# traupach/xarray_parcel

Hardware: AMD Instinct MI355X
Metric: column-profiles/sec for surface_based_cape_cin (higher is better)
Workload: dtype f64; 1 GPU; c2: synthetic 64-level x 1024 x 1024 f64 soundings per GPU, 64 levels x 1 x 1024 x 1024, surface_based_cape_cin (CAPE/CIN only), moist mode family, inputs resident in HBM; columns_total=1048576, columns_this_rank=1048576, levels=64, multi_gpu=single GPU

## Files before the change

### xarray_parcel_amd/csrc/xp_device.hpp

```cpp
#pragma once
#include <hip/hip_runtime.h>
#include <stdint.h>

namespace xp {

constexpr double RD = 287.04749097718457;
constexpr double EPS = 0.6219569100577033;
constexpr double KAPPA = 2.0 / 7.0;
constexpr double CP_D = RD / KAPPA;
constexpr double LV = 2.50084e6;
constexpr double G = 9.80665;
constexpr double VT_EPS = 0.608;
constexpr double RK4_H_MAX = 0.1;
constexpr double LCL_SNAP = 1e-11;

#define XP_DEV __device__ __forceinline__

XP_DEV double qnan() { return __longlong_as_double(0x7ff8000000000000LL); }
XP_DEV bool isnan_(double x) { return x != x; }
XP_DEV bool isclose_(double x, double y) { return fabs(x - y) <= 1e-8 + 1e-5 * fabs(y); }

constexpr int ST_TOP_NAN = 1, ST_LCL_NOT_CONVERGED = 2, ST_NAN_PRESSURE = 4, ST_BAD_PRESSURE = 8, ST_NO_LAYER = 16,
              ST_BAD_HEIGHT = 32, ST_LAYER_OPEN = 64;

// ... 273 lines not shown
    double es_td = es_ref(td);
    double w = EPS * es_td / (p_start - es_td);
    double p0 = p_start, p = qnan();
    bool conv = false;
    for (int it = 0; it < 50; ++it) {
        double td1 = log(p0 * w / (EPS + w) / 6.112); td1 = 273.15 + 243.5 * td1 / (17.67 - td1);
        double p1 = p_start * pow(td1 / t, 1.0 / KAPPA);
        double td2 = log(p1 * w / (EPS + w) / 6.112); td2 = 273.15 + 243.5 * td2 / (17.67 - td2);
        double p2 = p_start * pow(td2 / t, 1.0 / KAPPA);
        double d = p2 - 2.0 * p1 + p0;
        p = (d != 0.0) ? p0 - (p1 - p0) * (p1 - p0) / d : p2;
        double rel = (p0 != 0.0) ? (p - p0) / p0 : p;
        if (fabs(rel) < 1e-5) { conv = true; break; }
        p0 = p;
    }
    if (!conv) { p = qnan(); r.not_converged = 1; }
    if (fabs(p - p_start) <= 1e-8 + 1e-5 * fabs(p_start)) p = p_start;
    r.p = p;
    double v = log(p * w / (EPS + w) / 6.112);
    r.t = 273.15 + 243.5 * v / (17.67 - v);
    r.tv = virt_ref(r.t, r.t, p);
    return r;
}
__device__ __attribute__((noinline)) Lcl lcl_reference(double p_start, double t, double td) { return lcl_reference_body(p_start, t, td); }
template <bool FLAT = false> XP_DEV Lcl lcl(double p_start, double t, double td) {
    Lcl r;
    r.not_converged = 0;
    if (isnan_(p_start) || isnan_(t) || isnan_(td)) { r.p = r.t = r.tv = qnan(); return r; }
    bool sane = (td <= t) && (td > 150.0) && (t < 350.0) && (p_start > 50.0) && (p_start < 1200.0);
    double es_td = sat_vapor_pressure(td);
    double w = EPS * fdiv(es_td, p_start - es_td);
    double p0 = p_start, p = qnan();
    bool conv = false;
    for (int it = 0; it < 50; ++it) {
        double p1 = lcl_iter(p0, p_start, w, t);
        double p2 = lcl_iter(p1, p_start, w, t);
        double d = p2 - 2.0 * p1 + p0;
        p = (d != 0.0) ? p0 - fdiv((p1 - p0) * (p1 - p0), d) : p2;
        double rel = (p0 != 0.0) ? fdiv(p - p0, p0) : p;
        if (fabs(rel) < 1e-5) { conv = true; break; }
        p0 = p;
        if (!sane) break;
    }
    if (!conv) { p = qnan(); r.not_converged = 1; }
    if (fabs(p - p_start) <= 1e-8 + 1e-5 * fabs(p_start)) p = p_start;
    r.p = p;
    r.t = dewpoint_fast(p * fdiv(w, EPS + w));
    r.tv = virt(r.t, mix_of_e(sat_vapor_pressure(r.t), p));
    bool ref_path = !sane || (p == p_start);
    if (__builtin_amdgcn_ballot_w64(ref_path) != 0ull && ref_path) r = FLAT ? lcl_reference_body(p_start, t, td) : lcl_reference(p_start, t, td);
    return r;
}

XP_DEV double dt_dlnp_e(double p, double t, double e) {
    double pe = p - e, rt2 = RD * t * t;
    double num = __builtin_fma(RD * t, pe, (LV * EPS) * e);
    double den = __builtin_fma(CP_D * rt2, pe, (LV * LV * EPS * EPS) * e);
    return rt2 * fdiv(num, den);
}
XP_DEV double dt_dlnp(const double *es, double p, double t, bool fast) { return dt_dlnp_e(p, t, es_tab(es, t, fast)); }

struct Tables {
    const uint16_t *index;
    const float *adiabats;
    int64_t n_p, n_t;
    double p_max, p_step, t_min, t_step;
};

struct Moist {
    double x, p, t, e;
    const float *row;
    const double *es;
    bool table, dead;

    XP_DEV void start(const double *es_lds, double p_ref, double x_ref, double t_ref, bool table_mode, const Tables &tb) {
        es = es_lds; x = x_ref; p = p_ref; t = t_ref; table = table_mode; row = nullptr;
        e = es_tab(es, t_ref);
        dead = isnan_(p_ref) || isnan_(t_ref);
        if (table_mode && !dead) {
            double fi = (tb.p_max - p_ref) / tb.p_step, fj = (t_ref - tb.t_min) / tb.t_step;
            double i0 = floor(fi), j0 = floor(fj);
            int64_t ip = (int64_t)(((i0 + 1.0) - fi < fi - i0) ? i0 + 1.0 : i0);
            int64_t jt = (int64_t)(((j0 + 1.0) - fj <= fj - j0) ? j0 + 1.0 : j0);
            ip = ip < 0 ? 0 : (ip > tb.n_p - 1 ? tb.n_p - 1 : ip);
            jt = jt < 0 ? 0 : (jt > tb.n_t - 1 ? tb.n_t - 1 : jt);
            uint16_t a = tb.index[ip * tb.n_t + jt];
            if (a) row = tb.adiabats + (int64_t)(a - 1) * tb.n_p;
        }
    }
    XP_DEV double at(double pk, double xk, const Tables &tb, bool hoist = false) {
        if (dead || isnan_(pk)) return qnan();
        if (table) {
            double p_min = tb.p_max - (double)(tb.n_p - 1) * tb.p_step;
            if (row == nullptr || pk < p_min || pk > tb.p_max) return qnan();
            double f = (pk - p_min) / tb.p_step;
            int64_t lo = (int64_t)floor(f);
            if (lo >= tb.n_p - 1) return (double)row[tb.n_p - 1];
            double xlo = p_min + (double)lo * tb.p_step, xhi = p_min + (double)(lo + 1) * tb.p_step;
            double ylo = (double)row[lo], yhi = (double)row[lo + 1];
            return (yhi - ylo) / (xhi - xlo) * (pk - xlo) + ylo;
        }
        if (xk != x) {
            double dx = xk - x;
            int ns = (int)ceil(fabs(dx) * (1.0 / RK4_H_MAX) - 1e-12);
            ns = ns < 1 ? 1 : ns;
            double h = dx * frcp((double)ns);
            double q = 0.5 * h;
            double rh = 2.48015873015873e-05;
            rh = __builtin_fma(rh, q, 1.984126984126984e-04);
            rh = __builtin_fma(rh, q, 1.388888888888889e-03);
            rh = __builtin_fma(rh, q, 8.333333333333333e-03);
            rh = __builtin_fma(rh, q, 4.1666666666666664e-02);
            rh = __builtin_fma(rh, q, 1.6666666666666666e-01);
            rh = __builtin_fma(rh, q, 0.5);
            rh = __builtin_fma(rh, q, 1.0);
            rh = __builtin_fma(rh, q, 1.0);
            double ps = p;
            for (int s = 0; s < ns; ++s) {
                double pm = ps * rh;
                double pe = (s == ns - 1) ? pk : pm * rh;
                bool fast = hoist && (__builtin_amdgcn_ballot_w64(!in_table(t, 10.0)) == 0ull);
                double k1 = dt_dlnp_e(ps, t, e);
                double k2 = dt_dlnp(es, pm, t + 0.5 * h * k1, fast);
                double k3 = dt_dlnp(es, pm, t + 0.5 * h * k2, fast);
                double k4 = dt_dlnp(es, pe, t + h * k3, fast);
                t = t + (h * (1.0 / 6.0)) * (k1 + 2.0 * k2 + 2.0 * k3 + k4);
                e = es_tab(es, t, fast);
                ps = pe;
            }
            x = xk; p = pk;
        }
        return t;
    }
};

constexpr double FAM_XHI = 7.003065458786462;
constexpr double FAM_WX = 0.5, FAM_X1000 = 6.907755278982137;
constexpr int FAM_NPX = 8, FAM_ND = 8, FAM_MD = 8, FAM_NPS = 9;
constexpr double FAM_XLO = FAM_XHI - FAM_WX * FAM_NPX;
constexpr int FAM_COEFS = FAM_NPX * (FAM_ND + 1) * (FAM_MD + 1) * FAM_NPS;
constexpr int FAM_SIZE = FAM_COEFS + 2 * FAM_NPS;
constexpr double FAM_LABEL_H = 0.25, FAM_MARGIN = 0.05;
constexpr double FAM_PSI_LO = 215.0, FAM_PSI_HI = 312.0;
#define XP_FAM_EDGES {215.0, 245.0, 262.0, 275.0, 285.0, 293.0, 299.0, 304.0, 308.5, 312.0}

constexpr int FAM_SM = (FAM_ND + 1) * FAM_NPX * FAM_NPS, FAM_SN = FAM_NPX * FAM_NPS, FAM_SJ = FAM_NPS;
struct Family {
    const double *tab;
    double c[FAM_ND + 1];
    double m4;
    double s;
    int q;
    bool bad;

    XP_DEV static int psi_piece(double psi) {
        return (int)(psi >= 245.0) + (int)(psi >= 262.0) + (int)(psi >= 275.0) + (int)(psi >= 285.0) + (int)(psi >= 293.0) +
               (int)(psi >= 299.0) + (int)(psi >= 304.0) + (int)(psi >= 308.5);
    }
    XP_DEV static double x_mid(int j) { return FAM_XHI - FAM_WX * ((double)j + 0.5); }
    XP_DEV void load_piece(int j) {
        const double *a = tab + (j * FAM_SJ + q);
#pragma unroll
        for (int n = 0; n <= FAM_ND; ++n) {
            const double *r = a + n * FAM_SN;
            double k[FAM_MD + 1];
#pragma unroll
            for (int m = 0; m <= FAM_MD; ++m) k[m] = r[m * FAM_SM];
            lds_wait_all();
            double v = k[FAM_MD];
#pragma unroll
            for (int m = FAM_MD - 1; m >= 0; --m) v = __builtin_fma(v, s, k[m]);
            asm volatile("" : "+v"(v) : : "memory");
            c[n] = v;
        }
        m4 = -(2.0 / FAM_WX) * x_mid(j);
    }
    XP_DEV static double temperature_of(const double *es, double p, double tv) {
        constexpr double c = VT_EPS * EPS;
        double e0 = es_tab(es, tv);
        double t = fdiv(tv, 1.0 + c * fdiv(e0, p - e0));
#pragma nounroll
        for (int it = 0; it < 5; ++it) {
            double e = es_tab(es, t);
            double rt = frcp(t - 29.65), rp = frcp(p - e);
            double de = e * (17.67 * 243.5) * (rt * rt);
            double g = c * e * rp;
            double f = __builtin_fma(t, g, t) - tv;
            double df = 1.0 + g + t * c * p * de * (rp * rp);
            t = t - fdiv(f, df);
        }
        return t;
    }
    XP_DEV static double temperature_from(const double *es, double p, double tv, double &off, bool all_in_range = false) {
        constexpr double c = VT_EPS * EPS;
        double t = tv - off, f = 0.0;
#pragma nounroll
        for (int it = 0; it < 3; ++it) {
            double e = es_tab(es, t, all_in_range);
#ifdef XP_NEWTON_EXACT_SLOPE
            double rt = frcp(t - 29.65), rp = frcp(p - e);
#else
            double rt = __builtin_amdgcn_rcp(t - 29.65), rp = frcp(p - e);
#endif
            double de = e * (17.67 * 243.5) * (rt * rt);
            double g = c * e * rp;
            f = __builtin_fma(t, g, t) - tv;
            double df = 1.0 + g + t * c * p * de * (rp * rp);
#ifdef XP_NEWTON_EXACT_SLOPE
            t = t - fdiv(f, df);
#else
            t = t - f * __builtin_amdgcn_rcp(df);
#endif
        }
        bool more = !(fabs(f) <= 1e-6);
        if (__builtin_amdgcn_ballot_w64(more && !isnan_(tv)) != 0ull) {
#pragma nounroll
            for (int it = 0; it < 2; ++it) {
                double e = es_tab(es, t);
                double rt = frcp(t - 29.65), rp = frcp(p - e);
                double de = e * (17.67 * 243.5) * (rt * rt);
                double g = c * e * rp;
                double f2 = __builtin_fma(t, g, t) - tv;
                double df = 1.0 + g + t * c * p * de * (rp * rp);
                t = more ? t - fdiv(f2, df) : t;
            }
        }
        if (!isnan_(t)) off = tv - t;
        return t;
    }
    XP_DEV static double temperature_from2(const double *es, double p, double tv, double &off, double &offp, bool all_in_range) {
        constexpr double c = VT_EPS * EPS;
        double t = tv - (2.0 * off - offp), f = 0.0;
#pragma nounroll
        for (int it = 0; it < 2; ++it) {
            double e = es_tab(es, t, all_in_range);
            double rt = __builtin_amdgcn_rcp(t - 29.65), rp = frcp(p - e);
            double de = e * (17.67 * 243.5) * (rt * rt);
            double g = c * e * rp;
            f = __builtin_fma(t, g, t) - tv;
            double df = 1.0 + g + t * c * p * de * (rp * rp);
            t = t - f * __builtin_amdgcn_rcp(df);
        }
        bool more = !(fabs(f) <= 3e-5);
        if (__builtin_amdgcn_ballot_w64(more && !isnan_(tv)) != 0ull) {
#pragma nounroll
            for (int it = 0; it < 2; ++it) {
                double e = es_tab(es, t);
                double rt = frcp(t - 29.65), rp = frcp(p - e);
                double de = e * (17.67 * 243.5) * (rt * rt);
                double g = c * e * rp;
                double f2 = __builtin_fma(t, g, t) - tv;
                double df = 1.0 + g + t * c * p * de * (rp * rp);
                t = more ? t - fdiv(f2, df) : t;
            }
        }
        if (!isnan_(t)) { offp = off; off = tv - t; }
        return t;
    }
    XP_DEV double horner(double z) const {
        double v = c[FAM_ND];
#pragma unroll
        for (int n = FAM_ND - 1; n >= 0; --n) v = __builtin_fma(v, z, c[n]);
        return v;
    }
    XP_DEV void start(const double *table, const double *es, double p_lcl, double x_lcl, double t_lcl, double tv_lcl) {
        tab = table; q = 0; s = 0.0; m4 = 0.0;
        bad = !(x_lcl >= FAM_XLO && x_lcl <= FAM_XHI) || isnan_(t_lcl);
        double dx = FAM_X1000 - x_lcl;
        int ns = (int)ceil(fabs(dx) * (1.0 / FAM_LABEL_H) - 1e-12);
        ns = ns < 1 ? 1 : ns;
        ns = bad ? 1 : ns;
        double h = bad ? 0.0 : dx * frcp((double)ns);
        double qh = 0.5 * h;
        double rh = 2.755731922398589e-07;
        rh = __builtin_fma(rh, qh, 2.7557319223985893e-06);
        rh = __builtin_fma(rh, qh, 2.48015873015873e-05);
        rh = __builtin_fma(rh, qh, 1.984126984126984e-04);
        rh = __builtin_fma(rh, qh, 1.388888888888889e-03);
        rh = __builtin_fma(rh, qh, 8.333333333333333e-03);
        rh = __builtin_fma(rh, qh, 4.1666666666666664e-02);
        rh = __builtin_fma(rh, qh, 1.6666666666666666e-01);
        rh = __builtin_fma(rh, qh, 0.5);
        rh = __builtin_fma(rh, qh, 1.0);
        rh = __builtin_fma(rh, qh, 1.0);
        double t = t_lcl, ps = p_lcl;
#pragma nounroll
        for (int k = 0; k < ns; ++k) {
            double pm = ps * rh, pe = pm * rh;
            double k1 = dt_dlnp(es, ps, t, false);
            double k2 = dt_dlnp(es, pm, t + 0.5 * h * k1, false);
            double k3 = dt_dlnp(es, pm, t + 0.5 * h * k2, false);
            double k4 = dt_dlnp(es, pe, t + h * k3, false);
            t = t + (h * (1.0 / 6.0)) * (k1 + 2.0 * k2 + 2.0 * k3 + k4);
            ps = pe;
        }
        const double psi0 = t;
        if (!(psi0 >= FAM_PSI_LO + FAM_MARGIN && psi0 <= FAM_PSI_HI - FAM_MARGIN)) bad = true;
        q = bad ? 0 : psi_piece(psi0);
        const double mid = tab[FAM_COEFS + q], inv_h = tab[FAM_COEFS + FAM_NPS + q];
        double u = __builtin_fma(-(1.0 / FAM_WX), x_lcl, FAM_XHI * (1.0 / FAM_WX));
        int j0 = bad ? 0 : (int)u;
        j0 = j0 > FAM_NPX - 1 ? FAM_NPX - 1 : j0;
        const double z = bad ? 0.0 : (x_lcl - x_mid(j0)) * (2.0 / FAM_WX);
        const double *a = tab + (j0 * FAM_SJ + q);
        double b[FAM_MD + 1];
#pragma unroll
        for (int m = 0; m <= FAM_MD; ++m) {
            double k[FAM_ND + 1];
#pragma unroll
            for (int n = 0; n <= FAM_ND; ++n) k[n] = a[m * FAM_SM + n * FAM_SN];
            lds_wait_all();
            double v = k[FAM_ND];
#pragma unroll
            for (int n = FAM_ND - 1; n >= 0; --n) v = __builtin_fma(v, z, k[n]);
            asm volatile("" : "+v"(v) : : "memory");
            b[m] = v;
        }
        double psi = psi0;
#pragma unroll
        for (int it = 0; it < 3; ++it) {
            double sc = (psi - mid) * inv_h;
            double val = 0.0, der = 0.0;
#pragma unroll
            for (int m = FAM_MD; m >= 0; --m) {
                der = __builtin_fma(der, sc, val);
                val = __builtin_fma(val, sc, b[m]);
            }
            psi = psi - fdiv(val - tv_lcl, der * inv_h);
        }
        if (!(fabs(psi - psi0) <= FAM_MARGIN)) bad = true;
        s = bad ? 0.0 : (psi - mid) * inv_h;
        load_piece(j0);
        if (bad) poison();
    }
    XP_DEV double locate(double X, bool &top, bool &any_top) {
        double z = __builtin_fma(2.0 / FAM_WX, X, m4);
        top = false; any_top = false;
        bool move = (z <= -1.0) || (z > 1.0);
        if (__builtin_amdgcn_ballot_w64(move) != 0ull) {
            double u = __builtin_fma(-(1.0 / FAM_WX), X, FAM_XHI * (1.0 / FAM_WX));
            bool go = move;
            if (go && u < 0.0) { bad = true; go = false; }
            int jn = (int)u;
            top = go && jn > FAM_NPX - 1;
            int jcur = (int)__builtin_rint(__builtin_fma(m4, 0.5, FAM_XHI * (1.0 / FAM_WX) - 0.5));
            int j = go ? (jn > FAM_NPX - 1 ? FAM_NPX - 1 : jn) : jcur;
            load_piece(bad ? 0 : j);
            if (bad) poison();
            z = __builtin_fma(2.0 / FAM_WX, X, m4);
            any_top = __builtin_amdgcn_ballot_w64(top) != 0ull;
        }
        return z;
    }
    XP_DEV double top_value(double v, double X, bool top) const {
        const double w = horner(-1.0);
        return top ? w * fexp(KAPPA * (X - FAM_XLO)) : v;
    }
    XP_DEV double at(double X) {
        double z = __builtin_fma(2.0 / FAM_WX, X, m4);
        bool move = (z <= -1.0) || (z > 1.0);
        if (__builtin_amdgcn_ballot_w64(move) != 0ull) {
            double u = __builtin_fma(-(1.0 / FAM_WX), X, FAM_XHI * (1.0 / FAM_WX));
            bool go = move;
            if (go && u < 0.0) { bad = true; go = false; }
            int jn = (int)u;
            bool top = go && jn > FAM_NPX - 1;
            int jcur = (int)__builtin_rint(__builtin_fma(m4, 0.5, FAM_XHI * (1.0 / FAM_WX) - 0.5));
            int j = go ? (jn > FAM_NPX - 1 ? FAM_NPX - 1 : jn) : jcur;
            load_piece(bad ? 0 : j);
            if (bad) poison();
            z = __builtin_fma(2.0 / FAM_WX, X, m4);
            if (__builtin_amdgcn_ballot_w64(top) != 0ull) {
                double v = horner(top ? -1.0 : z);
                return top ? v * fexp(KAPPA * (X - FAM_XLO)) : v;
            }
        }
        return horner(z);
    }
    XP_DEV void poison() {
#pragma unroll
        for (int n = 0; n <= FAM_ND; ++n) c[n] = qnan();
        m4 = qnan();
    }
};

#ifndef XP_CAPE_THREADS
#define XP_CAPE_THREADS 256
#endif
#ifndef XP_SLOT_FIELDS
#define XP_SLOT_FIELDS (XP_CAPE_THREADS >= 1024 ? 12 : 13)
#endif
constexpr int SLOT_STRIDE = XP_CAPE_THREADS, SLOT_FIELDS = XP_SLOT_FIELDS;
enum { SL_CAPE_LCL = 0, SL_CIN_LCL, SL_MIN_P, SL_IDX , SL_LCL_T,
       SL_A0, SL_A1, SL_A2, SL_A3, SL_EL_X, SL_EL_T, SL_CAPE_EL, SL_LI ,
       SL_BR_P = SL_A0, SL_BR_X = SL_A1, SL_BR_T = SL_A2, SL_BR_TD = SL_A3,
       SL_LFC_X = SL_A0, SL_LFC_T = SL_A1, SL_CAPE_LFC = SL_A2, SL_CIN_LFC = SL_A3 };

struct Scan {
    double p_lcl, x_lcl;
    bool pos_neg;
    double *slot;
    double Xp, yp, parp;
    int j;
    bool use_all;
    double cape, cin;
    int any_inc;
    bool pos_parcel, env_any;
    bool top_le, any_valid;
    bool bad_p;

    XP_DEV void init(double p_lcl_, double x_lcl_, bool pos_neg_, double *slot_) {
        p_lcl = p_lcl_; x_lcl = x_lcl_; pos_neg = pos_neg_; slot = slot_;
        Xp = yp = parp = qnan(); j = 0; use_all = true;
        cape = cin = 0.0;
        for (int f = 0; f < SLOT_FIELDS; ++f)
            slot[f * SLOT_STRIDE] = (f == SL_LFC_T || f == SL_EL_T || f == SL_LFC_X || f == SL_EL_X || f == SL_MIN_P || f == SL_LI) ? qnan() : 0.0;
        idx()[0] = -1; idx()[1] = -1;
        any_inc = 0;
        pos_parcel = env_any = top_le = any_valid = bad_p = false;
    }
    XP_DEV int *idx() const { return (int *)(slot + SL_IDX * SLOT_STRIDE); }
    XP_DEV void add(double a) {
        if (pos_neg) { cape += fmax(a, 0.0); cin += fmin(a, 0.0); }
        else { double b = isnan_(a) ? 0.0 : a; cape += b; cin += b; }
    }
    XP_DEV double crossing_pressure(double xs) const {
        double ps = fexp(xs);
        bool near_lcl = fabs(xs - x_lcl) <= 2e-9;
        if (__builtin_amdgcn_ballot_w64(near_lcl) != 0ull && near_lcl) {
            double q = xs;
            asm volatile("" : "+v"(q));
            ps = exp_slow(q);
        }
        return ps;
    }
    template <bool LEAN, bool ABOVE> XP_DEV void special(double X, double par, double env, double y, double a_reg) {
        if (!ABOVE && j == 0) { use_all = (env != par); return; }
        int i = j - 1;
        double d = y - yp, xs, frac;
        if constexpr (ABOVE) {
            const double r = frcp1(d);
            xs = (y * Xp - yp * X) * r;
            if (isnan_(xs)) return;
            frac = -yp * r;
            add((yp * 0.5) * fabs(Xp - xs));
            if (y > 0.0) {
                any_inc = 1;
                if (!(xs <= slot[SL_LFC_X * SLOT_STRIDE])) {
                    slot[SL_LFC_X * SLOT_STRIDE] = xs; if (!LEAN) idx()[0] = j - 1;
                    if (!LEAN) slot[SL_LFC_T * SLOT_STRIDE] = frac * (par - parp) + parp;
                    slot[SL_CAPE_LFC * SLOT_STRIDE] = cape; slot[SL_CIN_LFC * SLOT_STRIDE] = cin;
                }
            }
            if (y < 0.0 && !(xs >= slot[SL_EL_X * SLOT_STRIDE])) {
                slot[SL_EL_X * SLOT_STRIDE] = xs; if (!LEAN) idx()[1] = j - 1;
                if (!LEAN) slot[SL_EL_T * SLOT_STRIDE] = frac * (par - parp) + parp;
                slot[SL_CAPE_EL * SLOT_STRIDE] = cape;
            }
            add((y * 0.5) * fabs(X - xs));
            return;
        }
        bool dup = (X == Xp);
        if (__builtin_amdgcn_ballot_w64(dup) != 0ull && dup) {
            xs = (y * Xp - yp * X) / d;
            frac = (xs - Xp) / (X - Xp);
        } else {
            double r = frcp1(d);
            xs = (y * Xp - yp * X) * r;
            frac = -yp * r;
        }
        double zy = frac * d + yp;
        if (isnan_(zy)) { add(a_reg); return; }
        double zlog = xs;
        bool above = ABOVE || xs < x_lcl;
        bool near_lcl = !ABOVE && fabs(xs - x_lcl) <= 2e-9;
        if (!ABOVE && __builtin_amdgcn_ballot_w64(near_lcl) != 0ull && near_lcl) {
            double q = y;
            asm volatile("" : "+v"(q));
            xs = crossing_x_ref(q, yp, X, Xp);
            double ps = exp_slow(xs);
            zlog = log_slow(ps);
            above = ps < p_lcl;
        }
        add((yp * 0.5) * fabs(Xp - zlog));
        double ys = frac * (par - parp) + parp;
        if (!isnan_(xs)) {
            bool in_sel = ABOVE || use_all || i >= 1;
            if (y > 0.0 && in_sel) {
                any_inc = 1;
                if (above && !(xs <= slot[SL_LFC_X * SLOT_STRIDE])) {
                    slot[SL_LFC_X * SLOT_STRIDE] = xs; if (!LEAN) idx()[0] = i;
                    if (!LEAN) slot[SL_LFC_T * SLOT_STRIDE] = ys;
                    slot[SL_CAPE_LFC * SLOT_STRIDE] = cape; slot[SL_CIN_LFC * SLOT_STRIDE] = cin;
                }
            }
            if (y < 0.0 && (ABOVE || i >= 1) && above && !(xs >= slot[SL_EL_X * SLOT_STRIDE])) {
                slot[SL_EL_X * SLOT_STRIDE] = xs; if (!LEAN) idx()[1] = i;
                if (!LEAN) slot[SL_EL_T * SLOT_STRIDE] = ys;
                slot[SL_CAPE_EL * SLOT_STRIDE] = cape;
            }
        }
        add((y * 0.5) * fabs(X - zlog));
    }
    template <bool LEAN = false, bool ABOVE = false> XP_DEV void node(double P, double X, double par, double env, bool is_lcl) {
        if (is_lcl) {
            slot[SL_LFC_X * SLOT_STRIDE] = qnan(); slot[SL_LFC_T * SLOT_STRIDE] = qnan();
            slot[SL_CAPE_LFC * SLOT_STRIDE] = 0.0; slot[SL_CIN_LFC * SLOT_STRIDE] = 0.0;
        }
        asm volatile("" : "+v"(par), "+v"(env));
        double y = par - env;
        bool same = (y * yp > 0.0) | ((y == 0.0) & (yp == 0.0));
        double a = fabs(X - Xp) * ((yp + y) * 0.5);
        add(same ? a : 0.0);
#ifdef XP_NODE_BALLOT
        if (__builtin_amdgcn_ballot_w64(!same) != 0ull && !same) special<LEAN, ABOVE>(X, par, env, y, a);
#else
        if (!same) special<LEAN, ABOVE>(X, par, env, y, a);
#endif
        pos_parcel = pos_parcel || ((ABOVE || P < p_lcl) && par > env);
        if (!LEAN) {
            bad_p = bad_p || (X > Xp);
            env_any = env_any || !isnan_(env);
        }
        bool pv = (ABOVE && LEAN) || !isnan_(P);
        bool valid = pv && !isnan_(par) && !isnan_(env);
        if (!LEAN && pv) slot[SL_MIN_P * SLOT_STRIDE] = P;
        top_le = (valid & (par <= env)) | (!valid & top_le);
        if (!LEAN) any_valid = any_valid || valid;
        if (is_lcl) { slot[SL_CAPE_LCL * SLOT_STRIDE] = cape; slot[SL_CIN_LCL * SLOT_STRIDE] = cin; }
        Xp = X; yp = y; parp = par; ++j;
// ... 44 lines not shown
```

### xarray_parcel_amd/csrc/xp_kernels.hpp

```cpp
#pragma once
#include "xp_level_reader.hpp"
#include "xp_profile_out.hpp"

namespace xp {

struct CapeArgs {
    View p, t, td;
    int64_t nlev, ncol;
    const void *ex_p, *ex_t, *ex_td;
    double depth;
    int vtc, log_interp, pos_neg, post_zero, table_mode;
    int hum;
    int off32;
    Tables tb;
    const double *es_tab;
    const double *fam_tab;
    int32_t *flags;
    int persist;
    int only_flagged;
    ScalarsOut s;
    ProfileOut prof;
};

enum { PM_SURFACE = 0, PM_MU = 1, PM_ML = 2, PM_EXPLICIT = 3 };
// ... 102 lines not shown
        if (!isnan_(p) && p < top) {
            double lt = flog(top), cb = flog(pb), ca = flog(p);
            double th_a = t / fpow(p / 1000.0, KAPPA), w_a = sat_mix(p, td);
            double cb2 = cb, ca2 = ca, tha = th_a, wa = w_a;
            if (pb == top) { ca2 = cb; tha = thb; wa = wb; }
            double th_t = interp_rule(thb, tha, lt, cb2, ca2), w_t = interp_rule(wb, wa, lt, cb2, ca2);
            layer_mean_step(s_th, pp, thp, top, th_t);
            layer_mean_step(s_w, pp, wp, top, w_t);
            r.first = k; closed = true;
            break;
        }
        double th = t / fpow(p / 1000.0, KAPPA), w = sat_mix(p, td);
        if (k > 0) { layer_mean_step(s_th, pp, thp, p, th); layer_mean_step(s_w, pp, wp, p, w); }
        pp = p; thp = th; wp = w;
        if (!isnan_(p)) { pb = p; thb = th; wb = w; }
    }
    if (!closed) {
        double th_t = (pb == top) ? thb : qnan(), w_t = (pb == top) ? wb : qnan();
        layer_mean_step(s_th, pp, thp, top, th_t);
        layer_mean_step(s_w, pp, wp, top, w_t);
    }
    double dlay = fabs(top - bottom);
    double th_m = (1.0 / dlay) * s_th, w_m = (1.0 / dlay) * s_w;
    r.p = p_start;
    r.t = th_m * fpow(p_start / 1000.0, KAPPA);
    r.td = dewpoint_of_e(vapor_pressure(p_start, w_m));
    return r;
}

template <typename T, bool HUM> XP_DEV Parcel choose_parcel(const CapeArgs &a, int pmode, int64_t c, const double *es, const double depth) {
    Parcel pc;
    if (pmode == PM_SURFACE) {
        pc.p = ld<T>(a.p, 0, c); pc.t = ld<T>(a.t, 0, c); pc.td = as_dewpoint<HUM>(es, pc.p, pc.t, ld<T>(a.td, 0, c));
        pc.first = 0; pc.idx = 0; pc.prepend = false;
    } else if (pmode == PM_EXPLICIT) {
        pc.p = ld1<T>(a.ex_p, c); pc.t = ld1<T>(a.ex_t, c); pc.td = ld1<T>(a.ex_td, c);
        pc.first = 0; pc.idx = -1; pc.prepend = false;
    } else if (pmode == PM_MU) {
        pc = select_mu<T, HUM>(a, c, es, depth);
    } else {
        pc = select_ml<T, HUM>(a, c, es, depth);
    }
    return pc;
}

template <typename T, int PMODE, bool PROFILE, int MODE, bool HUM, bool DEF, bool LEAN, bool PERSIST>
__global__ __launch_bounds__(XP_CAPE_THREADS, (XP_CAPE_THREADS >= 1024 ? 4 : MODE == 2 ? 3 : PROFILE ? 4 : (PMODE == PM_SURFACE ? (HUM ? 3 : 1) : 4))) void k_cape_cin(CapeArgs a) {
    constexpr bool TABLE = (MODE == 1), FAMILY = (MODE == 2);
    constexpr bool LAZY = FAMILY && PROFILE && LEAN;
    struct Lds { double es[LDS_TAB]; double fam[FAMILY ? FAM_SIZE : 1]; double slot[SLOT_FIELDS * SLOT_STRIDE]; int next; };
    struct LdsRef { double *es, *fam, *slot; int *next; } lds;
    if constexpr (FAMILY && PROFILE) {
        __shared__ double l_es[LDS_TAB];
        __shared__ double l_fam[FAM_SIZE];
        __shared__ double l_slot[SLOT_FIELDS * SLOT_STRIDE];
        __shared__ int l_next;
        lds.es = l_es; lds.fam = l_fam; lds.slot = l_slot; lds.next = &l_next;
    } else {
        __shared__ Lds l;
        lds.es = l.es; lds.fam = l.fam; lds.slot = l.slot; lds.next = &l.next;
    }
    double *const s_es = lds.es;
    double *const s_fam = lds.fam;
    if (FAMILY) for (int i = threadIdx.x; i < FAM_SIZE; i += blockDim.x) s_fam[i] = a.fam_tab[i];
    int &s_next = *lds.next;
    if (PERSIST && threadIdx.x == 0) s_next = (int)(blockDim.x >> 6);
    int64_t c0 = (int64_t)blockIdx.x * blockDim.x + threadIdx.x;
    if (a.only_flagged) {
        int need = (c0 < a.ncol) ? a.flags[c0] : 0;
        if (!__syncthreads_or(need)) return;
        stage_es_table(a.es_tab, s_es);
        if (!need) return;
    } else {
        stage_es_table(a.es_tab, s_es);
        if (!PERSIST && c0 >= a.ncol) return;
    }
    const double *es = s_es;
    double *const s_slot = lds.slot;

    auto column = [&](const int64_t c) __attribute__((always_inline)) {
    const Parcel pc = choose_parcel<T, HUM>(a, PMODE, c, es, a.depth);

    const bool vtc = DEF || (a.vtc != 0), pos_neg = DEF || (a.pos_neg != 0), log_interp = DEF || (a.log_interp != 0);
    const bool need_w = vtc || PROFILE;
    const Lcl l = lcl(pc.p, pc.t, pc.td);
    int status = l.not_converged ? ST_LCL_NOT_CONVERGED : 0;
    const ScalarsOut &s = a.s;

    if (isnan_(l.p)) {
        if (PROFILE) ProfileSink<T, LAZY>::blank(a.prof, c);
        store_blank_column(s, c, pc, l, status);
        if (FAMILY) a.flags[c] = 0;
        return;
    }

    store_parcel_and_lcl(s, c, pc, l);
    const double vf_parcel = need_w ? virt_factor_tab(es, pc.t, pc.td, pc.p, false) : 1.0;
    const double x_lcl = log(l.p);
    const double x0 = (pc.p == l.p) ? x_lcl : log_tab<true>(es, pc.p);

    Scan sc; sc.init(l.p, x_lcl, pos_neg, s_slot + threadIdx.x);
    sc.slot[SL_LCL_T * SLOT_STRIDE] = vtc ? l.tv : l.t;
    Moist m;
    Family fam;
    if (FAMILY) fam.start(s_fam, es, l.p, x_lcl, l.t, l.tv);
    else m.start(es, l.p, x_lcl, l.t, TABLE, a.tb);
    double fam_off = l.tv - l.t;
    double fam_offp = fam_off;

    ProfileSink<T, LAZY> sink;
    constexpr bool TRACK = LEAN && PMODE == PM_ML;
    int last_k = -1, cur_k = -1;
    auto emit = [&](auto above, double P, double X, double tp, double tvp, double te, double tve, double tde, bool is_lcl) __attribute__((always_inline)) {
        if (PROFILE) sink.node(a.prof, c, es, sc, P, X, tp, tvp, te, tve, tde);
        if (TRACK) {
            if (!isnan_(P)) { last_k = (is_lcl || cur_k < 0) ? -1 : cur_k; if (is_lcl || cur_k < 0) sc.slot[SL_MIN_P * SLOT_STRIDE] = P; }
        }
        sc.template node<LEAN, decltype(above)::value>(P, X, vtc ? tvp : tp, vtc ? tve : te, is_lcl);
    };

    bool lcl_done = false;
    double *const br = sc.slot;
    clear_bracket(br);
    auto moist_node = [&](double P, double X, double T_, double m_, bool Q) __attribute__((always_inline)) {
        constexpr bool TRIO = FAMILY && LEAN && !PROFILE && !HUM && (PMODE == PM_SURFACE || PMODE == PM_EXPLICIT);
        bool f_top = false, f_any_top = false;
        const double fz = TRIO ? fam.locate(X, f_top, f_any_top) : 0.0;
        double tf = TRIO ? 0.0 : FAMILY ? fam.at(X) : m.at(P, X, a.tb, true);
        constexpr bool PARCEL_ES = TABLE;
        constexpr bool FAM_T = FAMILY && PROFILE;
        unsigned dist = table_dist(T_);
        if (!Q) dist = umax_(dist, table_dist(m_));
        if (PARCEL_ES && need_w) dist = umax_(dist, table_dist(tf));
        const bool in_range = all_in_table(dist) && (!FAM_T || LAZY || in_table(tf, 8.0));
        double ep = 0.0, tve, tpf = 0.0;
        if (__builtin_amdgcn_ballot_w64(!in_range) == 0ull) {
            if (need_w && !FAMILY) ep = PARCEL_ES ? es_tab(es, tf, true) : m.e;
            if constexpr (TRIO) {
                double e_td, e_t;
                es_tab2_horner(es, m_, T_, fam.c, fz, e_td, e_t, tf);
                tve = T_ * __builtin_fma(e_td * frcp1(P - e_t), VT_EPS * EPS, 1.0);
            } else {
            tve = !need_w ? T_ : Q ? virt(T_, (m_ > 0.0 && m_ < 1.0) ? fdiv(m_, 1.0 - m_) : qnan()) : virt_env_tab<LEAN && !PROFILE>(es, T_, m_, P, true);
            }
            if (FAM_T) tpf = LAZY ? qnan() : Family::temperature_from2(es, P, tf, fam_off, fam_offp, true);
        } else {
            if constexpr (TRIO) tf = fam.horner(fz);
            double tq = tf;
            asm volatile("" : "+v"(tq));
            if (need_w && !FAMILY) ep = PARCEL_ES ? es_tab(es, tq, false) : m.e;
            tve = !need_w ? T_ : Q ? virt(T_, (m_ > 0.0 && m_ < 1.0) ? fdiv(m_, 1.0 - m_) : qnan()) : virt_env_tab(es, T_, m_, P, false);
            if (FAM_T) tpf = LAZY ? qnan() : Family::temperature_from2(es, P, tq, fam_off, fam_offp, false);
        }
        if constexpr (TRIO) { if (f_any_top) tf = fam.top_value(tf, X, f_top); }
        double tp, tvp;
        if (FAMILY) {
            tvp = tf;
            tp = PROFILE ? tpf : !vtc ? Family::temperature_of(es, P, tf) : tf;
        } else {
            tp = tf;
            tvp = need_w ? virt(tp, mix_of_e(ep, P)) : tp;
        }
        emit(std::true_type{}, P, X, tp, tvp, T_, tve, m_, false);
    };
    double sP = qnan(), sT = qnan(), sM = qnan();
    constexpr bool PREP = HUM && PMODE == PM_ML;
    bool s_is_td = false;
    auto source = [&](auto raw, double Pc, double Tc, double Mc, bool last, int kc) __attribute__((always_inline)) {
        const bool skew = lcl_done;
        double P = skew ? sP : Pc, T_ = skew ? sT : Tc;
        const double M_ = skew ? sM : Mc;
        double Td_ = (decltype(raw)::value && !(PREP && skew && s_is_td)) ? as_dewpoint<HUM>(es, P, T_, M_) : M_;
        double X;
        snap_to_lcl(es, l.p, x_lcl, P, X);
        if (TRACK) cur_k = skew ? kc - 1 : kc;
        const bool cross = !skew && (last || P < l.p);
        if (!LEAN && isnan_(P) && !skew && !last) status |= ST_NAN_PRESSURE;
        double tp, tvp;
        if (!skew) {
            tp = pc.t * dry_factor(es, KAPPA * (X - x0));
            tvp = need_w ? tp * vf_parcel : tp;
        } else if (FAMILY) {
            tvp = fam.at(X);
            if (PROFILE && !LAZY) fam_offp = fam_off;
            tp = LAZY ? qnan() : PROFILE ? Family::temperature_from(es, P, tvp, fam_off) : !vtc ? Family::temperature_of(es, P, tvp) : tvp;
        } else {
            tp = m.at(P, X, a.tb);
            tvp = need_w ? virt(tp, mix_of_e(TABLE ? es_tab(es, tp) : m.e, P)) : tp;
        }
        if (cross) {
            double te, tde;
            lcl_environment(br, log_interp, l.p, x_lcl, P, X, T_, Td_, te, tde);
            const double lsel = br[SL_LCL_T * SLOT_STRIDE];
            P = l.p; X = x_lcl; T_ = te; Td_ = tde;
            tp = PROFILE ? l.t : lsel; tvp = PROFILE ? l.tv : lsel;
        }
        double tve = need_w ? virt_env_ranged<LEAN && !PROFILE>(es, T_, Td_, P) : T_;
        lcl_ties(need_w, cross, l.p == pc.p, P, l.p, tp, T_, Td_, [&]() __attribute__((always_inline)) { return FAMILY ? l.t : m.at(P, X, a.tb); }, tvp, tve);
        emit(std::false_type{}, P, X, tp, tvp, T_, tve, Td_, cross);
        if (!isnan_(P) && !skew && !cross) store_bracket(br, P, X, T_, Td_);
        lcl_done = skew || cross;
        sP = Pc; sT = Tc; sM = Mc;
        if (PREP) s_is_td = !decltype(raw)::value;
    };

    if (pc.prepend) source(std::false_type{}, pc.p, pc.t, pc.td, false, -1);
    constexpr bool SEARCH = PMODE == PM_MU || PMODE == PM_ML;
    int k = (int)pc.first;
    LevelReader<T> rd(a.p, a.t, a.td, c);
    const int nlev = (int)a.nlev;
    rd.start(k, nlev);
    constexpr bool Q = HUM && !PROFILE;
    for (; k <= nlev; ++k) {
        if (__ballot(!lcl_done || (PREP && s_is_td)) == 0ull) break;
        double P, T_, M_;
        rd.take(k + 1 < nlev, P, T_, M_);
        source(std::true_type{}, P, T_, M_, k >= nlev, k);
    }
    auto plain_walk = [&](int k_) __attribute__((always_inline)) {
        int rem = __builtin_amdgcn_readfirstlane(nlev - k_);
        if (rem > 0) rd.step_back();
#ifndef XP_NO_PREWAIT
        rd.wait();
#endif
        rd.put_back(sP, sT, sM);
        rem += 1;
        asm volatile("" : "+s"(rem));
        for (; rem > 0; --rem, ++k_) {
            double P, T_, M_;
            rd.peek(P, T_, M_);
            if (rem > 1) rd.request();
            if (TRACK) cur_k = k_ - 1;
            moist_node(P, log_tab<true>(es, P), T_, Q ? M_ : as_dewpoint<HUM>(es, P, T_, M_), Q);
        }
    };
    if constexpr (SEARCH) {
        const int resume = k;
        int ku = nlev + 1;
        for (int probe = 0; probe <= nlev; ++probe) if (__ballot(resume <= probe) != 0ull) { ku = probe; break; }
        rd.start(ku, nlev);
        int rem = nlev - ku;
        asm volatile("" : "+s"(rem));
        for (; rem >= 0; --rem, ++ku) {
            double Pn, Tn, Mn;
            rd.take(rem > 1, Pn, Tn, Mn);
            if (ku >= resume) {
                if (TRACK) cur_k = ku - 1;
                moist_node(sP, log_tab<true>(es, sP), sT, Q ? sM : as_dewpoint<HUM>(es, sP, sT, sM), Q);
                sP = Pn; sT = Tn; sM = Mn;
            }
        }
    } else {
        plain_walk(k);
    }
    if (TRACK) {
        if (last_k >= 0) sc.slot[SL_MIN_P * SLOT_STRIDE] = ld<T>(a.p, last_k, c);
    } else if (LEAN) {
        double pm = l.p;
        bool found = false;
        if constexpr (!SEARCH) {
            const double q = rd.peek_p();
            if (!isnan_(q)) { pm = (q < pm) ? q : pm; found = true; }
        }
        for (int kk = nlev - 1; kk >= (int)pc.first; --kk) {
            if (__ballot(!found) == 0ull) break;
            const double q = ld<T>(a.p, kk, c);
            if (!found && !isnan_(q)) { pm = (q < pm) ? q : pm; found = true; }
        }
        sc.slot[SL_MIN_P * SLOT_STRIDE] = pm;
    }
    if (PROFILE) sink.finish(a.prof, c);

    const auto late = late_kernargs<CapeArgs>();
    Scan::Result r = sc.finish(late->post_zero != 0);
    if (FAMILY) late->flags[c] = fam.bad ? 1 : 0;
    store_scan_result(late->s, c, r, status | r.status);
    };

    if (PERSIST) persistent_tiles(a.ncol, s_next, column);
    else column(c0);
}

template <typename T, int PMODE> __global__ __launch_bounds__(256) void k_select_parcel(CapeArgs a) {
    __shared__ double s_es[LDS_TAB];
    const double *es = stage_es_table(a.es_tab, s_es);
    int64_t c = (int64_t)blockIdx.x * blockDim.x + threadIdx.x;
    if (c >= a.ncol) return;
    Parcel pc = choose_parcel<T, false>(a, PMODE, c, es, a.depth);
    st(a.s.par_p, a.s.f64, c, pc.p); st(a.s.par_t, a.s.f64, c, pc.t); st(a.s.par_td, a.s.f64, c, pc.td);
    sti(a.s.parcel_idx, c, pc.idx);
}

template <typename T> __global__ __launch_bounds__(256)
void k_mixed_layer(View pv, View vv, int64_t nlev, int64_t ncol, double depth_in, void *out, int f64) {
    int64_t c = (int64_t)blockIdx.x * blockDim.x + threadIdx.x;
    if (c >= ncol) return;
    double bottom = qnan(), top = qnan(), s = 0.0, pp = qnan(), vp = qnan(), pb = qnan(), vb = qnan();
    bool closed = false;
    for (int64_t k = 0; k < nlev; ++k) {
        double p = ld<T>(pv, k, c), v = ld<T>(vv, k, c);
        if (isnan_(bottom) && !isnan_(p)) { bottom = p; top = bottom - depth_in; }
        if (!isnan_(p) && p < top) {
            double cb = flog(pb), ca = flog(p), va = v;
            if (pb == top) { ca = cb; va = vb; }
            layer_mean_step(s, pp, vp, top, interp_rule(vb, va, flog(top), cb, ca));
            closed = true;
            break;
        }
        if (k > 0) layer_mean_step(s, pp, vp, p, v);
        pp = p; vp = v;
        if (!isnan_(p)) { pb = p; vb = v; }
    }
    if (!closed) layer_mean_step(s, pp, vp, top, (pb == top) ? vb : qnan());
    st(out, f64, c, (1.0 / fabs(top - bottom)) * s);
}

template <typename T> __global__ __launch_bounds__(256)
void k_lcl(int64_t n, const void *p, const void *t, const void *td, void *op, void *ot, void *otv, int32_t *status) {
    int64_t c = (int64_t)blockIdx.x * blockDim.x + threadIdx.x;
    if (c >= n) return;
    Lcl l = lcl(ld1<T>(p, c), ld1<T>(t, c), ld1<T>(td, c));
    const int f64 = sizeof(T) == 8;
    st(op, f64, c, l.p); st(ot, f64, c, l.t); st(otv, f64, c, l.tv); sti(status, c, l.not_converged ? 2 : 0);
}

template <typename T> __global__ __launch_bounds__(256)
void k_dry_lapse(View pv, int64_t nlev, int64_t ncol, const void *pt, const void *pp, OutView out) {
    int64_t c = (int64_t)blockIdx.x * blockDim.x + threadIdx.x;
    if (c >= ncol) return;
    double t0 = ld1<T>(pt, c), p0 = qnan();
    if (pp) p0 = ld1<T>(pp, c);
    else for (int64_t k = 0; k < nlev; ++k) { double p = ld<T>(pv, k, c); if (!isnan_(p) && !(p <= p0)) p0 = p; }
    for (int64_t k = 0; k < nlev; ++k) {
        double p = ld<T>(pv, k, c);
        st(out.data, sizeof(T) == 8, k * out.ls + c * out.cs, t0 * fpow(p / p0, KAPPA));
    }
}

template <typename T> __global__ __launch_bounds__(256)
void k_moist_lapse(View pv, int64_t nlev, int64_t ncol, const void *pt, const void *pp, int table_mode, Tables tb,
                   const double *es_g, OutView out) {
    __shared__ double s_es[LDS_TAB];
    const double *es = stage_es_table(es_g, s_es);
    int64_t c = (int64_t)blockIdx.x * blockDim.x + threadIdx.x;
    if (c >= ncol) return;
    const int f64 = sizeof(T) == 8;
    double t0 = ld1<T>(pt, c);
    double p0 = pp ? ld1<T>(pp, c) : ld<T>(pv, 0, c);
    double x0 = flog(p0);
    Moist m; m.start(es, p0, x0, t0, table_mode != 0, tb);
    for (int64_t k = 0; k < nlev; ++k) {
        double p = ld<T>(pv, k, c);
        if (p <= p0) st(out.data, f64, k * out.ls + c * out.cs, m.at(p, flog(p), tb));
        else if (!(p > p0)) st(out.data, f64, k * out.ls + c * out.cs, qnan());
    }
    m.start(es, p0, x0, t0, table_mode != 0, tb);
    for (int64_t k = nlev - 1; k >= 0; --k) {
        double p = ld<T>(pv, k, c);
        if (p > p0) st(out.data, f64, k * out.ls + c * out.cs, m.at(p, flog(p), tb));
    }
}

template <typename T> __global__ __launch_bounds__(256)
void k_parcel_profile(View pv, int64_t nlev, int64_t ncol, const void *pp, const void *pt, const void *ptd,
                      int table_mode, Tables tb, const double *es_g, OutView ot, OutView otv, void *olp, void *olt,
                      void *oltv) {
    __shared__ double s_es[LDS_TAB];
    const double *es = stage_es_table(es_g, s_es);
    int64_t c = (int64_t)blockIdx.x * blockDim.x + threadIdx.x;
    if (c >= ncol) return;
    const int f64 = sizeof(T) == 8;
    double p0 = ld1<T>(pp, c), t0 = ld1<T>(pt, c), td0 = ld1<T>(ptd, c);
    Lcl l = lcl(p0, t0, td0);
    double w_parcel = mixing_ratio(t0, td0, p0);
    double x_lcl = flog(l.p);
    Moist m; m.start(es, l.p, x_lcl, l.t, table_mode != 0, tb);
    for (int64_t k = 0; k < nlev; ++k) {
        double P = ld<T>(pv, k, c);
        double tp, w;
        if (P >= l.p) {
            tp = t0 * fpow(P / p0, KAPPA);
            w = (P == l.p) ? mix_of_e(sat_vapor_pressure(m.at(P, x_lcl, tb)), P) : w_parcel;
        } else {
            tp = m.at(P, flog(P), tb);
            w = mix_of_e(sat_vapor_pressure(tp), P);
        }
        if (ot.data) st(ot.data, f64, k * ot.ls + c * ot.cs, tp);
        if (otv.data) st(otv.data, f64, k * otv.ls + c * otv.cs, virt(tp, w));
    }
    st(olp, f64, c, l.p); st(olt, f64, c, l.t); st(oltv, f64, c, l.tv);
}

template <typename T> __global__ __launch_bounds__(XP_CAPE_THREADS)
void k_lfc_el(View pv, View parv, View envv, int64_t nlev, int64_t ncol, const void *lcl_p, const void *lcl_t,
              ScalarsOut s) {
    int64_t c = (int64_t)blockIdx.x * blockDim.x + threadIdx.x;
    if (c >= ncol) return;
    double lp = ld1<T>(lcl_p, c), lt = ld1<T>(lcl_t, c);
    __shared__ double s_slot[SLOT_FIELDS * SLOT_STRIDE];
    Scan sc; sc.init(lp, log(lp), true, s_slot + threadIdx.x);
    sc.slot[SL_LCL_T * SLOT_STRIDE] = lt;
    for (int64_t k = 0; k < nlev; ++k) {
        double P = ld<T>(pv, k, c);
        sc.node(P, (P == lp) ? sc.x_lcl : flog(P), ld<T>(parv, k, c), ld<T>(envv, k, c), false);
    }
    Scan::Result r = sc.finish(false);
    s.cape = s.cin = nullptr;
    store_scan_result(s, c, r, r.status);
}

template <typename T> __global__ __launch_bounds__(256)
void k_cape_cin_base(View pv, View envv, View parv, int64_t nlev, int64_t ncol, const void *lfc_p, const void *el_p,
                     int pos_neg, int post_zero, void *cape, void *cin) {
    int64_t c = (int64_t)blockIdx.x * blockDim.x + threadIdx.x;
    if (c >= ncol) return;
    const int f64 = sizeof(T) == 8;
    double L = ld1<T>(lfc_p, c), E = ld1<T>(el_p, c);
    if (isnan_(E)) {
        for (int64_t k = 0; k < nlev; ++k) { double p = ld<T>(pv, k, c); if (!isnan_(p) && !(p >= E)) E = p; }
// ... 188 lines not shown
```

Before: 2.250 billion column-profiles/s.

## Prefetch next family piece coefficients to avoid wave-wide reloads on single-step moves

Adds a second coefficient buffer (c1) in the Family state that holds the next pressure piece. When lanes in a wavefront only step one piece up, the next piece is loaded once and lanes switch to it individually, rather than the whole wave reloading on every crossing. A new value() helper evaluates the next-piece polynomial for lanes already switched. Separately, the minimum-pressure scan reads the pressure view from late kernargs. This raises register pressure and adds extra ballots and horner evaluations on the hot path.

```diff
diff --git a/xarray_parcel_amd/csrc/xp_device.hpp b/xarray_parcel_amd/csrc/xp_device.hpp
--- a/xarray_parcel_amd/csrc/xp_device.hpp
+++ b/xarray_parcel_amd/csrc/xp_device.hpp
@@ -449,13 +449,24 @@
     double s;
     int q;
     bool bad;
+    double c1[FAM_ND + 1];
+    bool have1;
+    int on1;
 
     XP_DEV static int psi_piece(double psi) {
         return (int)(psi >= 245.0) + (int)(psi >= 262.0) + (int)(psi >= 275.0) + (int)(psi >= 285.0) + (int)(psi >= 293.0) +
                (int)(psi >= 299.0) + (int)(psi >= 304.0) + (int)(psi >= 308.5);
     }
     XP_DEV static double x_mid(int j) { return FAM_XHI - FAM_WX * ((double)j + 0.5); }
-    XP_DEV void load_piece(int j) {
+    XP_DEV void load_piece(int j) { load_piece_into(j, c, m4); }
+    XP_DEV bool on() const { int o = on1; asm volatile("" : "+v"(o)); return o != 0; }
+    XP_DEV double m4_next() const {
+        double m = m4;
+        asm volatile("" : "+v"(m));
+        const double jd = __builtin_rint(__builtin_fma(m, 0.5, FAM_XHI * (1.0 / FAM_WX) - 0.5));
+        return -(2.0 / FAM_WX) * (FAM_XHI - FAM_WX * ((jd + 1.0) + 0.5));
+    }
+    XP_DEV void load_piece_into(int j, double *cc, double &mm) const {
         const double *a = tab + (j * FAM_SJ + q);
 #pragma unroll
         for (int n = 0; n <= FAM_ND; ++n) {
@@ -468,9 +479,9 @@
 #pragma unroll
             for (int m = FAM_MD - 1; m >= 0; --m) v = __builtin_fma(v, s, k[m]);
             asm volatile("" : "+v"(v) : : "memory");
-            c[n] = v;
-        }
-        m4 = -(2.0 / FAM_WX) * x_mid(j);
+            cc[n] = v;
+        }
+        mm = -(2.0 / FAM_WX) * x_mid(j);
     }
     XP_DEV static double temperature_of(const double *es, double p, double tv) {
         constexpr double c = VT_EPS * EPS;
@@ -561,7 +572,7 @@
         return v;
     }
     XP_DEV void start(const double *table, const double *es, double p_lcl, double x_lcl, double t_lcl, double tv_lcl) {
-        tab = table; q = 0; s = 0.0; m4 = 0.0;
+        tab = table; q = 0; s = 0.0; m4 = 0.0; have1 = false; on1 = 0;
         bad = !(x_lcl >= FAM_XLO && x_lcl <= FAM_XHI) || isnan_(t_lcl);
         double dx = FAM_X1000 - x_lcl;
         int ns = (int)ceil(fabs(dx) * (1.0 / FAM_LABEL_H) - 1e-12);
@@ -633,21 +644,61 @@
     XP_DEV double locate(double X, bool &top, bool &any_top) {
         double z = __builtin_fma(2.0 / FAM_WX, X, m4);
         top = false; any_top = false;
+        double z1 = z;
         bool move = (z <= -1.0) || (z > 1.0);
+        if (have1) {
+            z1 = __builtin_fma(2.0 / FAM_WX, X, m4_next());
+            asm volatile("" : "+v"(z1));
+            const double zc = on() ? z1 : z;
+            move = (zc <= -1.0) || (zc > 1.0);
+        }
         if (__builtin_amdgcn_ballot_w64(move) != 0ull) {
             double u = __builtin_fma(-(1.0 / FAM_WX), X, FAM_XHI * (1.0 / FAM_WX));
-            bool go = move;
-            if (go && u < 0.0) { bad = true; go = false; }
             int jn = (int)u;
-            top = go && jn > FAM_NPX - 1;
             int jcur = (int)__builtin_rint(__builtin_fma(m4, 0.5, FAM_XHI * (1.0 / FAM_WX) - 0.5));
-            int j = go ? (jn > FAM_NPX - 1 ? FAM_NPX - 1 : jn) : jcur;
-            load_piece(bad ? 0 : j);
-            if (bad) poison();
-            z = __builtin_fma(2.0 / FAM_WX, X, m4);
-            any_top = __builtin_amdgcn_ballot_w64(top) != 0ull;
+            const bool was1 = on();
+            const bool step = move && !was1 && !(u < 0.0) && jn == jcur + 1 && jn <= FAM_NPX - 1;
+            const bool plain = __builtin_amdgcn_ballot_w64(move && !step) == 0ull;
+            bool hand;
+            double m4_new;
+            if (plain && have1) {
+                const bool now1 = was1 || move;
+                on1 = now1 ? 1 : 0;
+                hand = __builtin_amdgcn_ballot_w64(!now1 && !bad) == 0ull;
+                m4_new = m4_next();
+            } else {
+                const bool next = plain && __builtin_amdgcn_ballot_w64(!move && !bad) != 0ull;
+                bool go = move && !next;
+                if (go && u < 0.0) { bad = true; go = false; }
+                top = go && jn > FAM_NPX - 1;
+                const int jhere = go ? jn : was1 ? jcur + 1 : jcur;
+                int j = next ? jcur + 1 : jhere;
+                j = j > FAM_NPX - 1 ? FAM_NPX - 1 : j;
+                load_piece_into(bad ? 0 : j, c1, m4_new);
+                if (bad) { poison1(); m4_new = qnan(); }
+                have1 = next; on1 = (next && move) ? 1 : 0;
+                hand = !next;
+                any_top = __builtin_amdgcn_ballot_w64(top) != 0ull;
+            }
+            if (hand) {
+#pragma unroll
+                for (int n = 0; n <= FAM_ND; ++n) c[n] = c1[n];
+                m4 = m4_new;
+                z = __builtin_fma(2.0 / FAM_WX, X, m4);
+                have1 = false; on1 = 0;
+            }
         }
         return z;
+    }
+    XP_DEV double value(double v, double X) const {
+        if (have1) {
+            const double z1 = __builtin_fma(2.0 / FAM_WX, X, m4_next());
+            double w = c1[FAM_ND];
+#pragma unroll
+            for (int n = FAM_ND - 1; n >= 0; --n) w = __builtin_fma(w, z1, c1[n]);
+            v = on() ? w : v;
+        }
+        return v;
     }
     XP_DEV double top_value(double v, double X, bool top) const {
         const double w = horner(-1.0);
@@ -673,6 +724,10 @@
             }
         }
         return horner(z);
+    }
+    XP_DEV void poison1() {
+#pragma unroll
+        for (int n = 0; n <= FAM_ND; ++n) c1[n] = qnan();
     }
     XP_DEV void poison() {
 #pragma unroll
diff --git a/xarray_parcel_amd/csrc/xp_kernels.hpp b/xarray_parcel_amd/csrc/xp_kernels.hpp
--- a/xarray_parcel_amd/csrc/xp_kernels.hpp
+++ b/xarray_parcel_amd/csrc/xp_kernels.hpp
@@ -278,7 +278,10 @@
             tve = !need_w ? T_ : Q ? virt(T_, (m_ > 0.0 && m_ < 1.0) ? fdiv(m_, 1.0 - m_) : qnan()) : virt_env_tab(es, T_, m_, P, false);
             if (FAM_T) tpf = LAZY ? qnan() : Family::temperature_from2(es, P, tq, fam_off, fam_offp, false);
         }
-        if constexpr (TRIO) { if (f_any_top) tf = fam.top_value(tf, X, f_top); }
+        if constexpr (TRIO) {
+            tf = fam.value(tf, X);
+            if (f_any_top) tf = fam.top_value(tf, X, f_top);
+        }
         double tp, tvp;
         if (FAMILY) {
             tvp = tf;
@@ -388,9 +391,11 @@
             const double q = rd.peek_p();
             if (!isnan_(q)) { pm = (q < pm) ? q : pm; found = true; }
         }
+        const auto late_in = late_kernargs<CapeArgs>();
+        const View top_p = {late_in->p.data, late_in->p.ls, late_in->p.cs};
         for (int kk = nlev - 1; kk >= (int)pc.first; --kk) {
             if (__ballot(!found) == 0ull) break;
-            const double q = ld<T>(a.p, kk, c);
+            const double q = ld<T>(top_p, kk, c);
             if (!found && !isnan_(q)) { pm = (q < pm) ? q : pm; found = true; }
         }
         sc.slot[SL_MIN_P * SLOT_STRIDE] = pm;
```

Result: faster. 2.327 billion column-profiles/s (median of 6 runs) (+3.4%).
